# yxlao/deepSpeech

Measured on AMD Instinct MI355X. Metric: audio-sec/sec training throughput (whole node), DS2 BiGRU, higher is better.
Workload: dtype bf16; 1 GPU; model=DeepSpeech2 2xconv(32) + 5xBiGRU-800 bidirectional + CTC, global_batch=32, seq_len=1000, parallelism=dp1, engine=hip

## Files before the change

deepspeech_amd/csrc/api.h:

```cpp
#pragma once
#include <hip/hip_runtime_api.h>
#include <stddef.h>

extern "C" {

struct DS2Fill {
  int n;
  unsigned* ptr[8];
  unsigned long long words[8];
  unsigned pattern[8];
};

hipEvent_t ds2_take_stop_event();
void ds2_arm_stop_event(hipEvent_t e);

int ds2_multi_fill(int n, void* const* ptrs, const unsigned long long* bytes, const unsigned* patterns,
                   hipStream_t st);
int ds2_multi_copy(int n, void* const* dst, const void* const* src, const unsigned long long* rows,
                   const unsigned* src_row, const unsigned* dst_row, const unsigned* src_pitch,
                   const unsigned* dst_pitch, float* sdst, const float* svals, int ns, hipStream_t st);
int ds2_wait_resident(const unsigned* word, long long timeout, hipStream_t st);
int ds2_prep_inputs(const float* x, void* y, long long n, const int* lens_in, int* lens_out, int nl,
                    hipStream_t st);
int ds2_transpose_bf16(const void* in, void* out, int R, int C, int ldi, int ldo, hipStream_t st);
// ... 166 lines not shown

int ds2_bn_stats(const void* y, int y_bf16, int N, int C, int T, int F, float* part, int nb, float eps, float* mean,
                 float* invstd, float* run_mean, float* run_var, float momentum, hipStream_t st);
int ds2_bn_chunks(int N, int T, int F);
int ds2_bn_apply(const void* y, int y_bf16, const float* mean, const float* invstd, const float* gamma,
                 const float* beta, void* out, int out_bf16, int N, int C, int T, int F, int layout, hipStream_t st);
int ds2_bn_bwd(const void* dout, int dout_bf16, const void* y, int y_bf16, const float* mean, const float* invstd,
               const float* gamma, const float* beta, float* part, int nb, float* dgamma, float* dbeta, void* dy,
               int dy_bf16, int N, int C, int T, int F, int layout, hipStream_t st);

int ds2_adam_ema(float* p, const float* g, float* m, float* v, float* ema, void* p16, long long n, float lr_t,
                 float b1, float b2, float eps, float gscale, float ema_keep, const int* skip, int max_grid,
                 const float* hyper, int lds_reserve, hipStream_t st);
int ds2_adam_ema_ranges(float* p, const float* g, float* m, float* v, float* ema, void* p16, const long long* lohi,
                        int nr, float lr_t, float b1, float b2, float eps, float gscale, float ema_keep,
                        const float* hyper, hipStream_t st);
int ds2_grad_norm_blocks(long long n);
int ds2_grad_norm(const float* g, long long n, float gscale, float* part, int nblocks, int* bad, hipStream_t st);
int ds2_cast_bf16(const float* x, void* y, long long n, hipStream_t st);
int ds2_col_sum(int n, const float* const* in, float* const* out, const int* R, const int* B, const int* C,
                const int* acc, hipStream_t st);
int ds2_fc_bias_grad(const void* G, int M, int ldg, int K, const float* scale, float alpha, float* out, int acc,
                     hipStream_t st);
int ds2_hist_nbucket();
int ds2_hist_npos();
int ds2_hist_blocks(long long n);
int ds2_hist_stats(const void* x, int bf16, long long n, unsigned* counts, float* part, int blocks, hipStream_t st);
int ds2_spin(long long ticks, int blocks, int threads, int lds_bytes, int* done, hipStream_t st);

struct DS2Conv1WgradBn {
  const void *dz, *y1;
  const float *mean, *invstd, *gamma, *beta, *dbeta, *dgamma;
};

struct DS2Conv2DgradBn {
  const void* y1;
  const float *mean, *invstd, *gamma, *beta;
  float* part;
};

size_t ds2_conv2_fwd_smem(int F1);
size_t ds2_conv2_dgrad_smem(int F2);
size_t ds2_conv2_wgrad_smem(int F1);
long long ds2_conv2_wgrad_part_floats(int grid);
long long ds2_conv1_wgrad_part_floats(int grid);
int ds2_conv1_fwd_grid(int N, int T1);
int ds2_conv1_fwd(const void* x, const void* w, const float* bias, void* y, float* part, int N, int T, int F0,
                  int T1, int F1, hipStream_t st);
int ds2_conv2_fwd(const void* x, const void* w, const float* bias, void* y, float* part, int grid, int N, int T1,
                  int F1, int T2, int F2, long long* trace, hipStream_t st);
int ds2_conv2_dgrad(const void* dy, const void* w, void* dx, int grid, int N, int T1, int F1, int T2, int F2,
                    const DS2Conv2DgradBn* bn, long long* trace, hipStream_t st);
int ds2_conv2_wgrad(const void* dy, const void* x, float* part, int grid, float* dw, int N, int T1, int F1, int T2,
                    int F2, hipStream_t st);
int ds2_conv1_wgrad(const void* dy, const void* x, float* part, int grid, float* dw, int N, int T, int F0, int T1,
                    int F1, const DS2Conv1WgradBn* bn, hipStream_t st);
int ds2_bn_cl_finalize(const float* part, int nb, double M, float eps, float* mean, float* invstd, float* run_mean,
                       float* run_var, float momentum, hipStream_t st);
int ds2_bn_cl_apply(const void* y, const float* mean, const float* invstd, const float* gamma, const float* beta,
                    void* out, int N, int T, int F, int tmaj, hipStream_t st);
int ds2_bn_cl_bwd(const void* dz, const void* y, const float* mean, const float* invstd, const float* gamma,
                  const float* beta, float* part, int nb, float* dgamma, float* dbeta, void* dy, int N, int T, int F,
                  int tmaj, int part_ready, hipStream_t st);

struct DS2Feat {
  const void* pcm;
  long long row_stride;
  int S, lead, mode, B, T_max;
  const int* lens;
  const float* offset;
  const float* gain;
  const float* basis;
  const int* mel_idx;
  const float* mel_w;
  const float* dct;
  const float* lifter;
  void* out;
  int* frames;
};

int ds2_audio_stats(const void* pcm, int in_i16, long long row_stride, int S, int B, const int* lens, float* offset,
                    float* gain, hipStream_t st);
int ds2_featurize(const DS2Feat* a, int kind, int in_i16, int out_bf16, hipStream_t st);

}
```

deepspeech_amd/csrc/bindings.cpp:

```cpp
#include <torch/extension.h>
#include <c10/hip/HIPStream.h>
#include <hip/hip_runtime.h>

#include <cstdint>
#include <string>
#include <vector>

#include "api.h"

namespace {

using OptT = c10::optional<at::Tensor>;

hipStream_t cur_stream() { return c10::hip::getCurrentHIPStream().stream(); }

void check(int rc, const char* what) {
  TORCH_CHECK(rc == 0, "deepspeech_amd kernel launch failed in ", what, " (code ", rc, ")");
}

constexpr unsigned kLightEvent = hipEventDisableTiming;

int64_t event_new(unsigned flags) {
  hipEvent_t e = nullptr;
  TORCH_CHECK(hipEventCreateWithFlags(&e, flags ? flags : kLightEvent) == hipSuccess, "hipEventCreateWithFlags");
// ... 454 lines not shown

void conv1_fwd(at::Tensor x, at::Tensor w, OptT bias, at::Tensor y, at::Tensor part) {
  need_bf16(x, "x"); need_bf16(w, "w"); need_bf16(y, "y");
  TORCH_CHECK(x.dim() == 3 && y.dim() == 4 && y.size(3) == 32 && w.numel() == 32 * 100, "conv1_fwd shapes");
  const int N = (int)x.size(0), T = (int)x.size(1), F0 = (int)x.size(2), T1 = (int)y.size(1), F1 = (int)y.size(2);
  TORCH_CHECK(y.size(0) == N, "conv1_fwd batch");
  need_f32(part, "part", (int64_t)ds2_conv1_fwd_grid(N, T1) * 64);
  check(ds2_conv1_fwd(x.data_ptr(), w.data_ptr(), ptr_or_null<float>(bias, "bias"), y.data_ptr(),
                      part.data_ptr<float>(), N, T, F0, T1, F1, cur_stream()), "conv1_fwd");
}
int64_t conv1_fwd_grid(int64_t N, int64_t T1) { return ds2_conv1_fwd_grid((int)N, (int)T1); }

long long* trace_ptr(const OptT& trace) {
  if (!trace) return nullptr;
  TORCH_CHECK(trace->is_cuda() && trace->scalar_type() == at::kLong && trace->numel() >= 8 * 16 * 6 &&
                  trace->is_contiguous(), "trace must be a contiguous cuda int64 tensor of >= 768 elements");
  return reinterpret_cast<long long*>(trace->data_ptr<int64_t>());
}

void conv2_fwd(at::Tensor x, at::Tensor w, OptT bias, at::Tensor y, at::Tensor part, int64_t grid, OptT trace) {
  need_bf16(x, "x"); need_bf16(w, "w"); need_bf16(y, "y");
  TORCH_CHECK(x.dim() == 4 && y.dim() == 4 && x.size(3) == 32 && y.size(3) == 32 && w.numel() == 32 * 32 * 50,
              "conv2_fwd shapes");
  TORCH_CHECK(grid > 0, "grid");
  need_f32(part, "part", grid * 64);
  check(ds2_conv2_fwd(x.data_ptr(), w.data_ptr(), ptr_or_null<float>(bias, "bias"), y.data_ptr(),
                      part.data_ptr<float>(), (int)grid, (int)x.size(0), (int)x.size(1), (int)x.size(2),
                      (int)y.size(1), (int)y.size(2), trace_ptr(trace), cur_stream()), "conv2_fwd");
}

void conv2_dgrad(at::Tensor dy, at::Tensor w, at::Tensor dx, int64_t grid, OptT y1, OptT mean, OptT invstd,
                 OptT gamma, OptT beta, OptT part, OptT trace) {
  need_bf16(dy, "dy"); need_bf16(w, "w"); need_bf16(dx, "dx");
  TORCH_CHECK(dy.dim() == 4 && dx.dim() == 4 && dy.size(3) == 32 && dx.size(3) == 32 && w.numel() == 32 * 32 * 50,
              "conv2_dgrad shapes");
  TORCH_CHECK(grid > 0, "grid");
  DS2Conv2DgradBn bn{};
  const bool with_bn = y1.has_value();
  if (with_bn) {
    TORCH_CHECK(mean && invstd && gamma && beta && part, "conv2_dgrad: the BN arguments come all or none");
    need_bf16(*y1, "y1");
    TORCH_CHECK(y1->sizes() == dx.sizes(), "y1 must have dx's shape");
    need_f32(*mean, "mean", 32); need_f32(*invstd, "invstd", 32); need_f32(*gamma, "gamma", 32);
    need_f32(*beta, "beta", 32); need_f32(*part, "part", grid * 64);
    bn = DS2Conv2DgradBn{y1->data_ptr(), mean->data_ptr<float>(), invstd->data_ptr<float>(),
                         gamma->data_ptr<float>(), beta->data_ptr<float>(), part->data_ptr<float>()};
  }
  check(ds2_conv2_dgrad(dy.data_ptr(), w.data_ptr(), dx.data_ptr(), (int)grid, (int)dx.size(0), (int)dx.size(1),
                        (int)dx.size(2), (int)dy.size(1), (int)dy.size(2), with_bn ? &bn : nullptr,
                        trace_ptr(trace), cur_stream()),
        "conv2_dgrad");
}

void conv2_wgrad(at::Tensor dy, at::Tensor x, at::Tensor part, at::Tensor dw, int64_t grid) {
  need_bf16(dy, "dy"); need_bf16(x, "x");
  TORCH_CHECK(grid > 0, "grid");
  need_f32(part, "part", ds2_conv2_wgrad_part_floats((int)grid));
  need_f32(dw, "dw", 32 * 32 * 50);
  check(ds2_conv2_wgrad(dy.data_ptr(), x.data_ptr(), part.data_ptr<float>(), (int)grid, dw.data_ptr<float>(),
                        (int)x.size(0), (int)x.size(1), (int)x.size(2), (int)dy.size(1), (int)dy.size(2),
                        cur_stream()), "conv2_wgrad");
}

void conv1_wgrad(at::Tensor dy, at::Tensor x, at::Tensor part, at::Tensor dw, int64_t grid, OptT y1, OptT mean,
                 OptT invstd, OptT gamma, OptT beta, OptT dbeta, OptT dgamma) {
  need_bf16(dy, "dy"); need_bf16(x, "x");
  TORCH_CHECK(grid > 0, "grid");
  need_f32(part, "part", ds2_conv1_wgrad_part_floats((int)grid));
  need_f32(dw, "dw", 32 * 100);
  DS2Conv1WgradBn bn{};
  const bool with_bn = y1.has_value();
  if (with_bn) {
    TORCH_CHECK(mean && invstd && gamma && beta && dbeta && dgamma, "conv1_wgrad: the BN arguments come all or none");
    need_bf16(*y1, "y1");
    TORCH_CHECK(y1->sizes() == dy.sizes(), "y1 must have dz's shape");
    for (const OptT* t : {&mean, &invstd, &gamma, &beta, &dbeta, &dgamma}) need_f32(**t, "bn vector", 32);
    bn = DS2Conv1WgradBn{dy.data_ptr(), y1->data_ptr(), mean->data_ptr<float>(), invstd->data_ptr<float>(),
                         gamma->data_ptr<float>(), beta->data_ptr<float>(), dbeta->data_ptr<float>(),
                         dgamma->data_ptr<float>()};
  }
  check(ds2_conv1_wgrad(with_bn ? nullptr : dy.data_ptr(), x.data_ptr(), part.data_ptr<float>(), (int)grid,
                        dw.data_ptr<float>(), (int)x.size(0), (int)x.size(1), (int)x.size(2), (int)dy.size(1),
                        (int)dy.size(2), with_bn ? &bn : nullptr, cur_stream()), "conv1_wgrad");
}
int64_t conv2_wgrad_part_floats(int64_t grid) { return ds2_conv2_wgrad_part_floats((int)grid); }
int64_t conv1_wgrad_part_floats(int64_t grid) { return ds2_conv1_wgrad_part_floats((int)grid); }

void bn_cl_finalize(at::Tensor part, int64_t nb, double M, double eps, at::Tensor mean, at::Tensor invstd,
                    OptT run_mean, OptT run_var, double momentum) {
  need_f32(part, "part", nb * 64);
  need_f32(mean, "mean", 32); need_f32(invstd, "invstd", 32);
  check(ds2_bn_cl_finalize(part.data_ptr<float>(), (int)nb, M, (float)eps, mean.data_ptr<float>(),
                           invstd.data_ptr<float>(), ptr_or_null<float>(run_mean, "run_mean"),
                           ptr_or_null<float>(run_var, "run_var"), (float)momentum, cur_stream()), "bn_cl_finalize");
}

void bn_cl_apply(at::Tensor y, at::Tensor mean, at::Tensor invstd, at::Tensor gamma, at::Tensor beta, at::Tensor out,
                 bool tmaj) {
  need_bf16(y, "y"); need_bf16(out, "out");
  TORCH_CHECK(y.dim() == 4 && y.size(3) == 32 && out.numel() == y.numel(), "bn_cl_apply shapes");
  need_f32(mean, "mean", 32); need_f32(invstd, "invstd", 32); need_f32(gamma, "gamma", 32); need_f32(beta, "beta", 32);
  check(ds2_bn_cl_apply(y.data_ptr(), mean.data_ptr<float>(), invstd.data_ptr<float>(), gamma.data_ptr<float>(),
                        beta.data_ptr<float>(), out.data_ptr(), (int)y.size(0), (int)y.size(1), (int)y.size(2),
                        tmaj ? 1 : 0, cur_stream()), "bn_cl_apply");
}

void bn_cl_bwd(at::Tensor dz, at::Tensor y, at::Tensor mean, at::Tensor invstd, at::Tensor gamma, at::Tensor beta,
               at::Tensor part, int64_t nb, at::Tensor dgamma, at::Tensor dbeta, at::Tensor dy, bool tmaj,
               int64_t part_ready) {
  need_bf16(dz, "dz"); need_bf16(y, "y"); need_bf16(dy, "dy");
  TORCH_CHECK(y.dim() == 4 && y.size(3) == 32 && dz.numel() == y.numel() && dy.numel() == y.numel(),
              "bn_cl_bwd shapes");
  need_f32(part, "part", nb * 64);
  need_f32(mean, "mean", 32); need_f32(invstd, "invstd", 32); need_f32(gamma, "gamma", 32); need_f32(beta, "beta", 32);
// ... 697 lines not shown
  m.def("bn_bwd", &bn_bwd);
  m.def("adam_ema", &adam_ema, py::arg("p"), py::arg("g"), py::arg("m"), py::arg("v"), py::arg("ema"),
        py::arg("p16"), py::arg("lr_t"), py::arg("b1"), py::arg("b2"), py::arg("eps"), py::arg("gscale"),
        py::arg("ema_keep"), py::arg("skip"), py::arg("max_grid"), py::arg("hyper") = py::none(),
        py::arg("lds_reserve") = 0);
  m.def("adam_ema_ranges", &adam_ema_ranges, py::arg("p"), py::arg("g"), py::arg("m"), py::arg("v"),
        py::arg("ema"), py::arg("p16"), py::arg("lohi"), py::arg("lr_t"), py::arg("b1"), py::arg("b2"),
        py::arg("eps"), py::arg("gscale"), py::arg("ema_keep"), py::arg("hyper") = py::none());
  m.def("grad_norm_blocks", &grad_norm_blocks);
  m.def("grad_norm", &grad_norm);
  m.def("cast_bf16", &cast_bf16);
  m.def("device_info", &device_info);
  m.def("fp8_quant_blocks", &fp8_quant_blocks);
  m.def("prep_inputs", &prep_inputs);
  m.def("multi_copy", &multi_copy, py::arg("dsts"), py::arg("srcs"), py::arg("sdst") = py::none(),
        py::arg("svals") = std::vector<double>{});
  m.def("fp8_quant2", &fp8_quant2, py::arg("a"), py::arg("b"), py::arg("alpha"), py::arg("a8"), py::arg("b8"),
        py::arg("part"), py::arg("scales"), py::arg("a2") = py::none(), py::arg("asum") = py::none());
  m.def("transpose_bf16", &transpose_bf16);
  m.def("gemm8", &gemm8, py::arg("A"), py::arg("B"), py::arg("C"), py::arg("bias"), py::arg("epi"),
        py::arg("alpha") = 1.0, py::arg("alpha_dev") = py::none(), py::arg("alpha_dev2") = py::none(),
        py::arg("a_col") = false, py::arg("b_col") = false, py::arg("splits") = 1, py::arg("ws") = py::none(),
        py::arg("cnt") = py::none(), py::arg("max_grid") = 0, py::arg("fill") = std::vector<at::Tensor>{},
        py::arg("fill_pat") = std::vector<int64_t>{}, py::arg("ext_red") = false);
  m.def("gemm8_group", &gemm8_group, py::arg("A"), py::arg("B"), py::arg("C"), py::arg("epi"), py::arg("splits"),
        py::arg("a_col"), py::arg("b_col"), py::arg("ws"), py::arg("cnt"), py::arg("max_grid"));
  m.def("gemm8_splits", [](int64_t K, bool fp8, int64_t S) { return ds2_gemm8_splits((int)K, fp8 ? 1 : 0, (int)S); });
  m.def("multi_fill", &multi_fill);
  m.def("col_sum", &col_sum);
  m.def("wait_resident", &wait_resident);
  m.def("fc_bias_grad", &fc_bias_grad);
  m.def("ctc_beam", &ctc_beam);
  m.def("ctc_beam_backtrack", &ctc_beam_backtrack);
  m.def("ctc_beam_lm", &ctc_beam_lm);
  m.def("ctc_beam_backtrack_lm", &ctc_beam_backtrack_lm);
  m.def("event_new", &event_new, py::arg("flags") = 0);
  m.def("arm_stop_event", &arm_stop_event);
  m.def("disarm_stop_event", &disarm_stop_event);
  m.def("event_free", &event_free);
  m.def("event_record", &event_record);
  m.def("event_wait", &event_wait);
  m.def("event_query", &event_query);
  m.def("stream_wait", &stream_wait);
  m.def("ctc_greedy", &ctc_greedy, py::arg("logits"), py::arg("lens"), py::arg("labels"), py::arg("counts"),
        py::arg("blank"), py::arg("score") = py::none());
  m.def("conv1_fwd", &conv1_fwd);
  m.def("conv1_fwd_grid", &conv1_fwd_grid);
  m.def("conv2_fwd", &conv2_fwd, py::arg("x"), py::arg("w"), py::arg("bias"), py::arg("y"), py::arg("part"),
        py::arg("grid"), py::arg("trace") = py::none());
  m.def("conv2_dgrad", &conv2_dgrad, py::arg("dy"), py::arg("w"), py::arg("dx"), py::arg("grid"),
        py::arg("y1") = py::none(), py::arg("mean") = py::none(), py::arg("invstd") = py::none(),
        py::arg("gamma") = py::none(), py::arg("beta") = py::none(), py::arg("part") = py::none(),
        py::arg("trace") = py::none());
  m.def("conv2_wgrad", &conv2_wgrad);
  m.def("conv1_wgrad", &conv1_wgrad, py::arg("dy"), py::arg("x"), py::arg("part"), py::arg("dw"), py::arg("grid"),
        py::arg("y1") = py::none(), py::arg("mean") = py::none(), py::arg("invstd") = py::none(),
        py::arg("gamma") = py::none(), py::arg("beta") = py::none(), py::arg("dbeta") = py::none(),
        py::arg("dgamma") = py::none());
  m.def("conv2_wgrad_part_floats", &conv2_wgrad_part_floats);
  m.def("conv1_wgrad_part_floats", &conv1_wgrad_part_floats);
  m.def("bn_cl_finalize", &bn_cl_finalize);
  m.def("bn_cl_apply", &bn_cl_apply);
  m.def("bn_cl_bwd", &bn_cl_bwd, py::arg("dz"), py::arg("y"), py::arg("mean"), py::arg("invstd"), py::arg("gamma"),
        py::arg("beta"), py::arg("part"), py::arg("nb"), py::arg("dgamma"), py::arg("dbeta"), py::arg("dy"),
        py::arg("tmaj"), py::arg("part_ready") = 0);
  m.def("gemm", &gemm, py::arg("A"), py::arg("B"), py::arg("C"), py::arg("bias"), py::arg("M"), py::arg("N"),
        py::arg("K"), py::arg("a_col"), py::arg("b_col"), py::arg("epi"), py::arg("alpha"), py::arg("cfg"),
        py::arg("alpha_dev") = py::none(), py::arg("Ml") = 0, py::arg("Nl") = 0, py::arg("Kl") = 0,
        py::arg("fill") = std::vector<at::Tensor>{}, py::arg("fill_pat") = std::vector<int64_t>{});
  m.def("gemm_tile", &gemm_tile);
  m.def("head_ctc", &head_ctc, py::arg("h"), py::arg("W"), py::arg("bias"), py::arg("lens"), py::arg("labels"),
        py::arg("label_lens"), py::arg("loss"), py::arg("G"), py::arg("ws"), py::arg("blank"), py::arg("zero_inf"),
        py::arg("mean") = py::none(), py::arg("counter") = py::none(), py::arg("first_bad") = py::none());
  m.def("fc_logits", &fc_logits);
  m.def("audio_stats", &audio_stats, py::arg("pcm"), py::arg("lens"), py::arg("offset"), py::arg("gain"));
  m.def("featurize", &featurize, py::arg("pcm"), py::arg("lens"), py::arg("offset"), py::arg("gain"),
        py::arg("basis"), py::arg("mel_idx"), py::arg("mel_w"), py::arg("dct"), py::arg("lifter"), py::arg("kind"),
        py::arg("lead"), py::arg("mode"), py::arg("out"), py::arg("frames"));
  m.def("hist_stats", &hist_stats);
  m.def("hist_nbucket", []() { return ds2_hist_nbucket(); });
  m.def("hist_blocks", [](int64_t n) { return ds2_hist_blocks(n); });
  m.def("nonfinite_watch", &nonfinite_watch);
  m.def("spin", [](int64_t ticks, int64_t blocks, int64_t threads, int64_t lds_bytes, at::Tensor done) {
    need_gpu(done, "done");
    TORCH_CHECK(done.scalar_type() == at::kInt, "done: int32");
    check(ds2_spin(ticks, (int)blocks, (int)threads, (int)lds_bytes, done.data_ptr<int>(), cur_stream()), "spin");
  });
}
```

deepspeech_amd/csrc/conv_frontend.hip:

```cpp
#include "common.h"

using namespace ds2;

namespace {

typedef __attribute__((ext_vector_type(16))) float f32x16;
typedef __attribute__((ext_vector_type(4))) short s16x4;
typedef __attribute__((address_space(3))) void lds_void_t;
typedef __attribute__((address_space(3))) s16x4 lds_s16x4_t;

constexpr int CC = 32;
constexpr float CLIP = 20.0f;
constexpr int MT = 3;

__device__ __forceinline__ f32x16 mfma32(bf16x8 a, bf16x8 b, f32x16 c) {
  return __builtin_amdgcn_mfma_f32_32x32x16_bf16(a, b, c, 0, 0, 0);
}

__device__ __forceinline__ void glds16(const void* g, void* lds_wave_base) {
  __builtin_amdgcn_global_load_lds(g, (lds_void_t*)lds_wave_base, 16, 0, 0);
}

__device__ __forceinline__ unsigned swz(unsigned R, unsigned c) { return R * 64u + ((c ^ ((R >> 2) & 3u)) << 4); }

// ... 352 lines not shown
#pragma unroll
          for (int j = 0; j < 2; ++j)
#pragma unroll
            for (int e = 0; e < 4; ++e) {
              const int fo = (32 * m + 8 * (2 * kh + j) + e) * CC;
              yv[m][j][e] = m < 2 ? yb[fo] : yb[min(fo, lastoff)];
            }
      }
#pragma unroll
      for (int m = 0; m < MT; ++m)
#pragma unroll
        for (int j = 0; j < 2; ++j)
#pragma unroll
          for (int e = 0; e < 4; ++e) {
            const int f1 = 32 * m + 8 * (2 * kh + j) + 4 * hi + e;
            if (m < 2 || f1 < a.F1) {
              const bf16_t d = f2bf(own[m][j][e]);
              stg[f1 * CC + col] = d;
              if (bn) {
                const float xh = (bf2f(yv[m][j][e]) - bmu) * bis;
                const float zz = xh * bg + bbt;
                const float dd = (zz > 0.f && zz < CLIP) ? bf2f(d) : 0.f;
                bs += dd;
                bq += dd * xh;
              }
            }
          }
    }
    lds_barrier();
    if (out) {
      i32x4* dst = (i32x4*)(a.dx + rowoff);
      for (int q = kh * 64 + lane; q < a.F1 * 4; q += 128) dst[q] = ((const i32x4*)stg)[q];
    }
    c2_stamp(a.trace, it, 4);
    if (tile + per < t_hi) issue(tile + per);
    c2_stamp(a.trace, it, 5);
  }
  if (bn) {
    bs += __shfl_xor(bs, 32, 64);
    bq += __shfl_xor(bq, 32, 64);
    float* sh = (float*)red;
    __syncthreads();
    if (lane < 32) { sh[(w * 32 + lane) * 2] = bs; sh[(w * 32 + lane) * 2 + 1] = bq; }
    __syncthreads();
    if (tid < 64) a.part[(size_t)blockIdx.x * 64 + tid] = sh[tid] + sh[64 + tid] + sh[128 + tid] + sh[192 + tid];
  }
}

struct Conv2Wgrad {
  const bf16_t* dy;
  const bf16_t* x;
  float* part;
  int N, T1, F1, T2, F2;
};
constexpr int C2W_PAIRS = C2_KT * C2_KF;
constexpr int C2W_WAVES = 8;
constexpr int C2W_PPW = 7;

__global__ __launch_bounds__(512) void conv2_wgrad_kernel(Conv2Wgrad a) {
  extern __shared__ __attribute__((aligned(16))) unsigned char smem[];
  const int tid = threadIdx.x, lane = tid & 63, w = uni(tid >> 6);
  const int dyBytes = 80 * 64;
  const int xBytes = (9 * a.F1 + 84) * 64;
  const int bufBytes = dyBytes + xBytes;
  unsigned char* const buf0 = smem;
  unsigned char* const buf1 = smem + bufBytes;
  for (int b = 0; b < 2; ++b) {
    unsigned char* bb = b ? buf1 : buf0;
    for (int o = a.F2 * 64 + tid * 4; o < dyBytes; o += 512 * 4) *(unsigned*)(bb + o) = 0u;
    for (int o = 10 * a.F1 * 64 + tid * 4; o < xBytes; o += 512 * 4) *(unsigned*)(bb + dyBytes + o) = 0u;
  }
  const int ntiles = a.N * a.T2;
  const int dyChunks = a.F2 * 4, xChunks = 10 * a.F1 * 4;
  auto issue = [&](int t, unsigned char* dst) {
    const int n = t / a.T2, t2 = t - n * a.T2;
    const unsigned char* sdy = (const unsigned char*)(a.dy + ((size_t)n * a.T2 + t2) * a.F2 * CC);
    const unsigned char* sx = (const unsigned char*)(a.x + ((size_t)n * a.T1 + 2 * t2) * a.F1 * CC);
    for (int p0 = w * 64; p0 < dyChunks; p0 += 512) {
      const int p = p0 + lane;
      if (p < dyChunks) glds16(sdy + (size_t)p * 16, dst + (size_t)p0 * 16);
    }
    for (int p0 = w * 64; p0 < xChunks; p0 += 512) {
      const int p = p0 + lane;
      if (p < xChunks) glds16(sx + (size_t)p * 16, dst + dyBytes + (size_t)p0 * 16);
    }
  };
  const int g = lane >> 4, h = g >> 1, cb = (g & 1) * 16, q = (lane & 15) >> 2, pp = lane & 3;
  const unsigned lofs = (unsigned)((8 * h + q) * 64 + (cb + 4 * pp) * 2);
  const int npairs = (w < C2W_PAIRS - 6 * C2W_WAVES) ? 7 : 6;

  f32x16 acc[C2W_PPW];
#pragma unroll
  for (int i = 0; i < C2W_PPW; ++i) acc[i] = (f32x16){};
  __syncthreads();
  int it = 0;
  if ((int)blockIdx.x < ntiles) issue(blockIdx.x, buf0);
  for (int tile = blockIdx.x; tile < ntiles; tile += gridDim.x, ++it) {
    const unsigned char* cur = (it & 1) ? buf1 : buf0;
    asm volatile("s_waitcnt vmcnt(0)" ::: "memory");
    __syncthreads();
    if (tile + (int)gridDim.x < ntiles) issue(tile + gridDim.x, (it & 1) ? buf0 : buf1);
    const unsigned char* xs = cur + dyBytes;
#pragma unroll
    for (int kk = 0; kk < 5; ++kk) {
      const unsigned k0 = (unsigned)(16 * kk) * 64u;
      const bf16x8 av = cat8(tr_read(cur + k0 + lofs), tr_read(cur + k0 + lofs + 4 * 64));
#pragma unroll
      for (int i = 0; i < C2W_PPW; ++i) {
        if (i < npairs) {
          const int P = w + C2W_WAVES * i;
          const int kt = P / 5, kf = P - 5 * (P / 5);
          const unsigned rb = (unsigned)(kt * a.F1 + kf) * 64u + k0 + lofs;
          const bf16x8 bv = cat8(tr_read(xs + rb), tr_read(xs + rb + 4 * 64));
          acc[i] = mfma32(av, bv, acc[i]);
        }
      }
    }
  }
  f32x4* out = (f32x4*)(a.part + (size_t)blockIdx.x * C2W_PAIRS * 1024);
#pragma unroll
  for (int i = 0; i < C2W_PPW; ++i) {
    if (i < npairs) {
      const int P = w + C2W_WAVES * i;
#pragma unroll
      for (int r4 = 0; r4 < 4; ++r4)
        out[(P * 4 + r4) * 64 + lane] = (f32x4){acc[i][4 * r4], acc[i][4 * r4 + 1], acc[i][4 * r4 + 2], acc[i][4 * r4 + 3]};
    }
  }
}

template <int KIND>
__global__ __launch_bounds__(256) void wgrad_reduce_kernel(const float* __restrict__ part, int nb, int E,
                                                           float* __restrict__ dw) {
  __shared__ f32x4 sh[4][64];
  const int tid = threadIdx.x, g = tid >> 6, l = tid & 63;
  const int e4 = blockIdx.x * 64 + l, E4 = E >> 2;
  const f32x4* p4 = (const f32x4*)part;
  f32x4 s0 = {}, s1 = {};
  int b = g;
  for (; b + 4 < nb; b += 8) {
    s0 += p4[(size_t)b * E4 + e4];
    s1 += p4[(size_t)(b + 4) * E4 + e4];
  }
  if (b < nb) s0 += p4[(size_t)b * E4 + e4];
  sh[g][l] = s0 + s1;
  __syncthreads();
  if (g != 0) return;
  const f32x4 v = sh[0][l] + sh[1][l] + sh[2][l] + sh[3][l];
#pragma unroll
  for (int j = 0; j < 4; ++j) {
    const int e = e4 * 4 + j;
    const int P = e >> 10, rem = e & 1023, r4 = rem >> 8, ln = (rem >> 2) & 63;
    const int row = (rem & 3) + 8 * r4 + 4 * (ln >> 5), c = ln & 31;
    if (KIND == 0) {
      const int kt = P / 5, kf = P % 5;
      dw[((row * CC + c) * C2_KT + kt) * C2_KF + kf] = v[j];
    } else {
      const int kt = 4 * P + (c >> 3), kf = c & 7;
      if (kf < 5) dw[(row * 20 + kt) * 5 + kf] = v[j];
    }
  }
}

struct Conv1Fwd {
  const bf16_t* x;
  const bf16_t* w;
  const float* bias;
  bf16_t* y;
  float* part;
  int N, T, F0, T1, F1;
// ... 42 lines not shown
  __syncthreads();
  float ssum = 0.f, ssq = 0.f;
  const int t1 = t1_0 + w;
  if (t1 < a.T1) {
    f32x16 acc[MT];
#pragma unroll
    for (int m = 0; m < MT; ++m) acc[m] = (f32x16){};
#pragma unroll
    for (int s = 0; s < 10; ++s) {
      const int r = 2 * w + 2 * s + hi;
#pragma unroll
      for (int m = 0; m < MT; ++m) {
        const unsigned* p = (const unsigned*)(xs + r * C1_XS + 2 * (32 * m + col));
        const unsigned u0 = p[0], u1 = p[1], u2 = p[2], u3 = p[3];
        const bf16x8 av = __builtin_bit_cast(bf16x8, (i32x4){(int)u0, (int)u1, (int)u2, (int)u3});
        acc[m] = mfma32(av, bfr[s], acc[m]);
      }
    }
    bf16_t* yl = ys[w];
#pragma unroll
    for (int m = 0; m < MT; ++m)
#pragma unroll
      for (int r = 0; r < 16; ++r) {
        const int f1 = 32 * m + (r & 3) + 8 * (r >> 2) + 4 * hi;
        if (f1 < a.F1) {
          const bf16_t b = f2bf(acc[m][r] + bco);
          yl[f1 * CC + col] = b;
          const float vb = bf2f(b);
          ssum += vb;
          ssq += vb * vb;
        }
      }
    i32x4* dst = (i32x4*)(a.y + ((size_t)n * a.T1 + t1) * a.F1 * CC);
    for (int q = lane; q < a.F1 * 4; q += 64) dst[q] = ((const i32x4*)yl)[q];
  }
  write_stats(ssum, ssq, statsh, 4, a.part);
}

struct Conv1Wgrad {
  const bf16_t* dy;
  const bf16_t* x;
  float* part;
  int N, T, F0, T1, F1;
  const bf16_t *dz, *y1;
  const float *mean, *invstd, *gamma, *beta, *dbeta, *dgamma;
  float M;
};
constexpr int C1W_XP = 88;
constexpr int C1W_DY = C1_ROWS * 80 * 64;
constexpr int C1W_XD = C1_IN * 8 * C1W_XP * 2;
constexpr int C1W_RED = 4 * 5 * 4 * 64 * 16;
constexpr int C1W_RAW = C1_IN * C1_XS * 2;
constexpr int C1W_SMEM = (C1W_DY + C1W_XD + C1W_RAW) > C1W_RED ? (C1W_DY + C1W_XD + C1W_RAW) : C1W_RED;

__global__ __launch_bounds__(256) void conv1_wgrad_kernel(Conv1Wgrad a) {
  extern __shared__ __attribute__((aligned(16))) unsigned char smem[];
  const int tid = threadIdx.x, lane = tid & 63, w = uni(tid >> 6);
  const int hi = lane >> 5, col = lane & 31;
  unsigned char* dys = smem;
  bf16_t* xd = (bf16_t*)(smem + C1W_DY);
  bf16_t* raw = (bf16_t*)(smem + C1W_DY + C1W_XD);
  const int tb = (a.T1 + C1_ROWS - 1) / C1_ROWS;
  const int ntiles = a.N * tb;
  const int g = lane >> 4, h = g >> 1, cb = (g & 1) * 16, q = (lane & 15) >> 2, pp = lane & 3;
  const unsigned lofs = (unsigned)((8 * h + q) * 64 + (cb + 4 * pp) * 2);
  const int bkt = col >> 3, bkf = col & 7;

  const bool bn = a.dz != nullptr;
  float bmu[8], bis[8], bg[8], bbt[8], bmdb[8], bmdg[8];
  if (bn) {
#pragma unroll
    for (int j = 0; j < 8; ++j) {
      const int c = (tid & 3) * 8 + j;
      bmu[j] = a.mean[c]; bis[j] = a.invstd[c]; bg[j] = a.gamma[c]; bbt[j] = a.beta[c];
      bmdb[j] = a.dbeta[c] / a.M; bmdg[j] = a.dgamma[c] / a.M;
    }
  }
  f32x16 acc[5];
#pragma unroll
  for (int i = 0; i < 5; ++i) acc[i] = (f32x16){};
  for (int tile = blockIdx.x; tile < ntiles; tile += gridDim.x) {
    const int n = tile / tb, t1_0 = (tile - n * tb) * C1_ROWS;
    __syncthreads();
    for (int ch = tid; ch < C1_ROWS * 80 * 4; ch += 256) {
      const int r = ch / 320, rem = ch - r * 320, pos = rem >> 2, c4 = rem & 3;
      const int t1 = t1_0 + r;
      i32x4 v = (i32x4){0, 0, 0, 0};
      if (pos < a.F1 && t1 < a.T1) {
        const size_t off = (((size_t)n * a.T1 + t1) * a.F1 + pos) * CC + c4 * 8;
        if (bn) {
          const bf16x8 y = *(const bf16x8*)(a.y1 + off), d = *(const bf16x8*)(a.dz + off);
          bf16x8 o;
#pragma unroll
          for (int j = 0; j < 8; ++j) {
            const float xh = (bf2f((bf16_t)y[j]) - bmu[j]) * bis[j];
            const float zz = xh * bg[j] + bbt[j];
            const float dd = (zz > 0.f && zz < CLIP) ? bf2f((bf16_t)d[j]) : 0.f;
            o[j] = (short)f2bf(bg[j] * bis[j] * (dd - bmdb[j] - xh * bmdg[j]));
          }
          v = __builtin_bit_cast(i32x4, o);
        } else {
          v = *(const i32x4*)(a.dy + off);
        }
      }
      *(i32x4*)(dys + ch * 16) = v;
    }
    stage_rows(raw, a.x + (size_t)n * a.T * a.F0, 2 * t1_0, a.T, a.F0);
    __syncthreads();
    for (int ch = tid; ch < C1_IN * 8 * 10; ch += 256) {
      const int kf = ch & 7, q = ch >> 3, r = q / 10, p0 = (q - r * 10) * 8;
      bf16x8 v;
#pragma unroll
      for (int j = 0; j < 8; ++j) v[j] = (short)raw[r * C1_XS + min(2 * (p0 + j) + kf, C1_XS - 1)];
      *(bf16x8*)(xd + (r * 8 + kf) * C1W_XP + p0) = v;
    }
    __syncthreads();
    const int t1 = t1_0 + w;
    if (t1 < a.T1) {
#pragma unroll
      for (int kk = 0; kk < 5; ++kk) {
        const unsigned k0 = (unsigned)(16 * kk);
        const unsigned char* ab = dys + (w * 80 + k0) * 64 + lofs;
        const bf16x8 av = cat8(tr_read(ab), tr_read(ab + 4 * 64));
#pragma unroll
        for (int nt = 0; nt < 5; ++nt) {
          const int r = 2 * w + 4 * nt + bkt;
          const bf16x8 bv = *(const bf16x8*)(xd + (r * 8 + bkf) * C1W_XP + k0 + 8 * hi);
          acc[nt] = mfma32(av, bv, acc[nt]);
        }
      }
    }
  }
  __syncthreads();
  f32x4* red = (f32x4*)smem;
#pragma unroll
  for (int nt = 0; nt < 5; ++nt)
#pragma unroll
    for (int r4 = 0; r4 < 4; ++r4)
      red[((w * 5 + nt) * 4 + r4) * 64 + lane] =
          (f32x4){acc[nt][4 * r4], acc[nt][4 * r4 + 1], acc[nt][4 * r4 + 2], acc[nt][4 * r4 + 3]};
  __syncthreads();
  f32x4* out = (f32x4*)(a.part + (size_t)blockIdx.x * 5 * 1024);
  for (int e = tid; e < 5 * 4 * 64; e += 256) {
    f32x4 v = red[e];
    for (int wv = 1; wv < 4; ++wv) v += red[wv * 5 * 4 * 64 + e];
    out[e] = v;
  }
}

__global__ __launch_bounds__(256) void bn_cl_finalize_kernel(const float* __restrict__ part, int nb, double M,
                                                             float eps, float* mean, float* invstd, float* run_mean,
                                                             float* run_var, float momentum) {
  __shared__ double sh[2][4];
  const int c = blockIdx.x, tid = threadIdx.x;
  double s = 0.0, q = 0.0;
  for (int b = tid; b < nb; b += 256) {
    s += part[((size_t)b * 32 + c) * 2 + 0];
    q += part[((size_t)b * 32 + c) * 2 + 1];
  }
#pragma unroll
  for (int o = 32; o > 0; o >>= 1) {
    s += __shfl_xor(s, o, 64);
    q += __shfl_xor(q, o, 64);
  }
  if ((tid & 63) == 0) { sh[0][tid >> 6] = s; sh[1][tid >> 6] = q; }
  __syncthreads();
  if (tid == 0) {
// ... 213 lines not shown
#pragma unroll
    for (int k = 0; k < 4; ++k) o8[e + k * step] = one(v[k], d[k]);
  }
  for (; e < total; e += step) o8[e] = one(y8[e], d8[e]);
}

template <typename K>
int set_smem(K kernel, size_t bytes) {
  return (int)hipFuncSetAttribute(reinterpret_cast<const void*>(kernel), hipFuncAttributeMaxDynamicSharedMemorySize,
                                  (int)bytes);
}

int shape_ok(int T1, int F1, int T2, int F2) {
  if (F1 < 5 || F1 > 80 || F2 != F1 - 4) return -40;
  if (T1 < 10 || T2 != (T1 - 10) / 2 + 1) return -41;
  return 0;
}

}

extern "C" {

size_t ds2_conv2_fwd_smem(int) { return (size_t)C2F_SMEM; }
size_t ds2_conv2_dgrad_smem(int) { return (size_t)C2D_SMEM; }
size_t ds2_conv2_wgrad_smem(int F1) { return (size_t)2 * (80 * 64 + (9 * F1 + 84) * 64); }
long long ds2_conv2_wgrad_part_floats(int grid) { return (long long)grid * C2W_PAIRS * 1024; }
long long ds2_conv1_wgrad_part_floats(int grid) { return (long long)grid * 5 * 1024; }
int ds2_conv1_fwd_grid(int N, int T1) { return N * ((T1 + C1_ROWS - 1) / C1_ROWS); }

int ds2_conv2_fwd(const void* x, const void* w, const float* bias, void* y, float* part, int grid, int N, int T1,
                  int F1, int T2, int F2, long long* trace, hipStream_t st) {
  if (int e = shape_ok(T1, F1, T2, F2)) return e;
  const size_t smem = ds2_conv2_fwd_smem(F1);
  DS2_HIP_CHECK((hipError_t)set_smem(conv2_fwd_kernel, smem));
  Conv2Fwd a{(const bf16_t*)x, (const bf16_t*)w, bias, (bf16_t*)y, part, N, T1, F1, T2, F2, trace};
  hipLaunchKernelGGL(conv2_fwd_kernel, dim3(grid), dim3(256), smem, st, a);
  return (int)hipGetLastError();
}

int ds2_conv2_dgrad(const void* dy, const void* w, void* dx, int grid, int N, int T1, int F1, int T2, int F2,
                    const DS2Conv2DgradBn* bn, long long* trace, hipStream_t st) {
  if (int e = shape_ok(T1, F1, T2, F2)) return e;
  if (F1 <= 64) return -42;
  const size_t smem = ds2_conv2_dgrad_smem(F2);
  DS2_HIP_CHECK((hipError_t)set_smem(conv2_dgrad_kernel, smem));
  Conv2Dgrad a{(const bf16_t*)dy, (const bf16_t*)w, (bf16_t*)dx, N, T1, F1, T2, F2,
               bn ? (const bf16_t*)bn->y1 : nullptr, bn ? bn->mean : nullptr, bn ? bn->invstd : nullptr,
               bn ? bn->gamma : nullptr, bn ? bn->beta : nullptr, bn ? bn->part : nullptr, trace};
  hipLaunchKernelGGL(conv2_dgrad_kernel, dim3(grid), dim3(256), smem, st, a);
  return (int)hipGetLastError();
}

int ds2_conv2_wgrad(const void* dy, const void* x, float* part, int grid, float* dw, int N, int T1, int F1, int T2,
                    int F2, hipStream_t st) {
  if (int e = shape_ok(T1, F1, T2, F2)) return e;
  const size_t smem = ds2_conv2_wgrad_smem(F1);
  DS2_HIP_CHECK((hipError_t)set_smem(conv2_wgrad_kernel, smem));
  Conv2Wgrad a{(const bf16_t*)dy, (const bf16_t*)x, part, N, T1, F1, T2, F2};
  hipLaunchKernelGGL(conv2_wgrad_kernel, dim3(grid), dim3(512), smem, st, a);
  hipLaunchKernelGGL(wgrad_reduce_kernel<0>, dim3(C2W_PAIRS * 1024 / 256), dim3(256), 0, st, part, grid,
                     C2W_PAIRS * 1024, dw);
  return (int)hipGetLastError();
}

int ds2_conv1_fwd(const void* x, const void* w, const float* bias, void* y, float* part, int N, int T, int F0,
                  int T1, int F1, hipStream_t st) {
  if (F1 > 96 || F1 != (F0 - 5) / 2 + 1 || T1 != (T - 20) / 2 + 1 || T1 < 1) return -42;
  Conv1Fwd a{(const bf16_t*)x, (const bf16_t*)w, bias, (bf16_t*)y, part, N, T, F0, T1, F1};
  hipLaunchKernelGGL(conv1_fwd_kernel, dim3(ds2_conv1_fwd_grid(N, T1)), dim3(256), 0, st, a);
  return (int)hipGetLastError();
}

int ds2_conv1_wgrad(const void* dy, const void* x, float* part, int grid, float* dw, int N, int T, int F0, int T1,
                    int F1, const DS2Conv1WgradBn* bn, hipStream_t st) {
  if (F1 > 80 || F1 != (F0 - 5) / 2 + 1 || T1 != (T - 20) / 2 + 1 || T1 < 1) return -43;
  if ((dy == nullptr) == (bn == nullptr)) return -44;
  DS2_HIP_CHECK((hipError_t)set_smem(conv1_wgrad_kernel, C1W_SMEM));
  Conv1Wgrad a{(const bf16_t*)dy, (const bf16_t*)x, part, N, T, F0, T1, F1,
               bn ? (const bf16_t*)bn->dz : nullptr, bn ? (const bf16_t*)bn->y1 : nullptr,
               bn ? bn->mean : nullptr, bn ? bn->invstd : nullptr, bn ? bn->gamma : nullptr,
               bn ? bn->beta : nullptr, bn ? bn->dbeta : nullptr, bn ? bn->dgamma : nullptr,
               (float)((double)N * T1 * F1)};
  hipLaunchKernelGGL(conv1_wgrad_kernel, dim3(grid), dim3(256), C1W_SMEM, st, a);
  hipLaunchKernelGGL(wgrad_reduce_kernel<1>, dim3(5 * 1024 / 256), dim3(256), 0, st, part, grid, 5 * 1024, dw);
  return (int)hipGetLastError();
}

int ds2_bn_cl_finalize(const float* part, int nb, double M, float eps, float* mean, float* invstd, float* run_mean,
                       float* run_var, float momentum, hipStream_t st) {
  hipLaunchKernelGGL(bn_cl_finalize_kernel, dim3(CC), dim3(256), 0, st, part, nb, M, eps, mean, invstd, run_mean,
                     run_var, momentum);
  return (int)hipGetLastError();
}

int ds2_bn_cl_apply(const void* y, const float* mean, const float* invstd, const float* gamma, const float* beta,
                    void* out, int N, int T, int F, int tmaj, hipStream_t st) {
  if (F > 96) return -44;
  if (tmaj) {
    const int rows = N * T;
    hipLaunchKernelGGL(bn_cl_apply_tmaj_kernel, dim3(rows < 4096 ? rows : 4096), dim3(256), 0, st, (const bf16_t*)y,
                       mean, invstd, gamma, beta, (bf16_t*)out, N, T, F);
  } else {
    const long long nch = (long long)N * T * F * 4;
    long long nb = (nch + 255) / 256;
    if (nb > 8192) nb = 8192;
    hipLaunchKernelGGL(bn_cl_apply_kernel, dim3((unsigned)nb), dim3(256), 0, st, (const bf16_t*)y, mean, invstd,
                       gamma, beta, (bf16_t*)out, nch);
  }
  return (int)hipGetLastError();
}

// ... 19 lines not shown
```

Measured before the change: 41950 audio-sec/sec.

## Prefetch next conv1 wgrad tile into registers and permute-based x deinterleave

The conv1 weight-gradient kernel now loads the next tile's dy/dz/y1 and raw input rows into registers while the current tile is processed, which hides global-load latency behind the MFMA work. The stride-2 deinterleave of input rows into the shared-memory layout now uses 32-bit reads and byte permutes in place of per-element gathers. Optional trace timestamps are also added to the conv2 wgrad kernel. The register double-buffer raises VGPR pressure and could lower occupancy, and the unaligned-read edge handling adds complexity.

```diff
diff --git a/deepspeech_amd/csrc/api.h b/deepspeech_amd/csrc/api.h
--- a/deepspeech_amd/csrc/api.h
+++ b/deepspeech_amd/csrc/api.h
@@ -242,7 +242,7 @@
 int ds2_conv2_dgrad(const void* dy, const void* w, void* dx, int grid, int N, int T1, int F1, int T2, int F2,
                     const DS2Conv2DgradBn* bn, long long* trace, hipStream_t st);
 int ds2_conv2_wgrad(const void* dy, const void* x, float* part, int grid, float* dw, int N, int T1, int F1, int T2,
-                    int F2, hipStream_t st);
+                    int F2, long long* trace, hipStream_t st);
 int ds2_conv1_wgrad(const void* dy, const void* x, float* part, int grid, float* dw, int N, int T, int F0, int T1,
                     int F1, const DS2Conv1WgradBn* bn, hipStream_t st);
 int ds2_bn_cl_finalize(const float* part, int nb, double M, float eps, float* mean, float* invstd, float* run_mean,
diff --git a/deepspeech_amd/csrc/bindings.cpp b/deepspeech_amd/csrc/bindings.cpp
--- a/deepspeech_amd/csrc/bindings.cpp
+++ b/deepspeech_amd/csrc/bindings.cpp
@@ -530,14 +530,14 @@
         "conv2_dgrad");
 }
 
-void conv2_wgrad(at::Tensor dy, at::Tensor x, at::Tensor part, at::Tensor dw, int64_t grid) {
+void conv2_wgrad(at::Tensor dy, at::Tensor x, at::Tensor part, at::Tensor dw, int64_t grid, OptT trace) {
   need_bf16(dy, "dy"); need_bf16(x, "x");
   TORCH_CHECK(grid > 0, "grid");
   need_f32(part, "part", ds2_conv2_wgrad_part_floats((int)grid));
   need_f32(dw, "dw", 32 * 32 * 50);
   check(ds2_conv2_wgrad(dy.data_ptr(), x.data_ptr(), part.data_ptr<float>(), (int)grid, dw.data_ptr<float>(),
                         (int)x.size(0), (int)x.size(1), (int)x.size(2), (int)dy.size(1), (int)dy.size(2),
-                        cur_stream()), "conv2_wgrad");
+                        trace_ptr(trace), cur_stream()), "conv2_wgrad");
 }
 
 void conv1_wgrad(at::Tensor dy, at::Tensor x, at::Tensor part, at::Tensor dw, int64_t grid, OptT y1, OptT mean,
@@ -1341,7 +1341,8 @@
         py::arg("y1") = py::none(), py::arg("mean") = py::none(), py::arg("invstd") = py::none(),
         py::arg("gamma") = py::none(), py::arg("beta") = py::none(), py::arg("part") = py::none(),
         py::arg("trace") = py::none());
-  m.def("conv2_wgrad", &conv2_wgrad);
+  m.def("conv2_wgrad", &conv2_wgrad, py::arg("dy"), py::arg("x"), py::arg("part"), py::arg("dw"), py::arg("grid"),
+        py::arg("trace") = py::none());
   m.def("conv1_wgrad", &conv1_wgrad, py::arg("dy"), py::arg("x"), py::arg("part"), py::arg("dw"), py::arg("grid"),
         py::arg("y1") = py::none(), py::arg("mean") = py::none(), py::arg("invstd") = py::none(),
         py::arg("gamma") = py::none(), py::arg("beta") = py::none(), py::arg("dbeta") = py::none(),
diff --git a/deepspeech_amd/csrc/conv_frontend.hip b/deepspeech_amd/csrc/conv_frontend.hip
--- a/deepspeech_amd/csrc/conv_frontend.hip
+++ b/deepspeech_amd/csrc/conv_frontend.hip
@@ -428,6 +428,7 @@
   const bf16_t* x;
   float* part;
   int N, T1, F1, T2, F2;
+  long long* trace;
 };
 constexpr int C2W_PAIRS = C2_KT * C2_KF;
 constexpr int C2W_WAVES = 8;
@@ -473,9 +474,12 @@
   if ((int)blockIdx.x < ntiles) issue(blockIdx.x, buf0);
   for (int tile = blockIdx.x; tile < ntiles; tile += gridDim.x, ++it) {
     const unsigned char* cur = (it & 1) ? buf1 : buf0;
+    c2_stamp(a.trace, it, 0);
     asm volatile("s_waitcnt vmcnt(0)" ::: "memory");
     __syncthreads();
+    c2_stamp(a.trace, it, 1);
     if (tile + (int)gridDim.x < ntiles) issue(tile + gridDim.x, (it & 1) ? buf0 : buf1);
+    c2_stamp(a.trace, it, 2);
     const unsigned char* xs = cur + dyBytes;
 #pragma unroll
     for (int kk = 0; kk < 5; ++kk) {
@@ -492,6 +496,7 @@
         }
       }
     }
+    c2_stamp(a.trace, it, 3);
   }
   f32x4* out = (f32x4*)(a.part + (size_t)blockIdx.x * C2W_PAIRS * 1024);
 #pragma unroll
@@ -640,6 +645,97 @@
 constexpr int C1W_RED = 4 * 5 * 4 * 64 * 16;
 constexpr int C1W_RAW = C1_IN * C1_XS * 2;
 constexpr int C1W_SMEM = (C1W_DY + C1W_XD + C1W_RAW) > C1W_RED ? (C1W_DY + C1W_XD + C1W_RAW) : C1W_RED;
+constexpr int C1W_CK = C1_ROWS * 80 * 4 / 256;
+static_assert(C1W_CK * 256 == C1_ROWS * 80 * 4, "a tile's dy chunks divide evenly over the workgroup");
+constexpr int C1W_XG = 21;
+constexpr int C1W_XN = C1_IN * C1W_XG;
+constexpr int C1W_XI = (C1W_XN + 255) / 256;
+static_assert(8 * C1W_XG > 2 * 79 + 7 && 8 * C1W_XG <= C1_XS, "staged columns cover what is read");
+
+struct C1wTile {
+  i32x4 d[C1W_CK];
+  i32x4 y[C1W_CK];
+  i32x4 x[C1W_XI];
+  unsigned x4[C1W_XI];
+};
+
+__device__ __forceinline__ bool c1w_xitem(const Conv1Wgrad& a, int n, int t0, int it, int& r, int& g,
+                                          const bf16_t*& row, uintptr_t& lo, bool& odd) {
+  r = it / C1W_XG;
+  g = it - r * C1W_XG;
+  row = a.x + ((size_t)n * a.T + min(t0 + r, a.T - 1)) * a.F0;
+  const uintptr_t ad = (uintptr_t)(row + 8 * g);
+  lo = ad & ~(uintptr_t)3;
+  odd = (ad & 2) != 0;
+  return lo >= (uintptr_t)a.x && lo + 20 <= (uintptr_t)(a.x + (size_t)a.N * a.T * a.F0);
+}
+
+__device__ __forceinline__ bool c1w_chunk(int ch, int t1_0, int T1, int F1, int& t1, int& pos, int& c4) {
+  const int r = ch / 320, rem = ch - r * 320;
+  pos = rem >> 2;
+  c4 = rem & 3;
+  t1 = t1_0 + r;
+  return pos < F1 && t1 < T1;
+}
+
+__device__ __forceinline__ void c1w_load(C1wTile& t, const Conv1Wgrad& a, int tile, int tb, bool bn) {
+  const int n = tile / tb, t1_0 = (tile - n * tb) * C1_ROWS;
+#pragma unroll
+  for (int k = 0; k < C1W_CK; ++k) {
+    int t1, pos, c4;
+    c1w_chunk((int)threadIdx.x + 256 * k, t1_0, a.T1, a.F1, t1, pos, c4);
+    const size_t off = (((size_t)n * a.T1 + min(t1, a.T1 - 1)) * a.F1 + min(pos, a.F1 - 1)) * CC + c4 * 8;
+    if (bn) {
+      t.y[k] = *(const i32x4*)(a.y1 + off);
+      t.d[k] = *(const i32x4*)(a.dz + off);
+    } else {
+      t.d[k] = *(const i32x4*)(a.dy + off);
+    }
+  }
+#pragma unroll
+  for (int k = 0; k < C1W_XI; ++k) {
+    const int it = (int)threadIdx.x + 256 * k;
+    if (it >= C1W_XN) continue;
+    int r, g;
+    const bf16_t* row;
+    uintptr_t lo;
+    bool odd;
+    if (c1w_xitem(a, n, 2 * t1_0, it, r, g, row, lo, odd)) {
+      t.x[k] = *(const i32x4*)lo;
+      t.x4[k] = *(const unsigned*)(lo + 16);
+    } else {
+      bf16x8 v;
+#pragma unroll
+      for (int j = 0; j < 8; ++j) v[j] = (short)row[min(8 * g + j, a.F0 - 1)];
+      t.x[k] = __builtin_bit_cast(i32x4, v);
+      t.x4[k] = 0;
+    }
+  }
+}
+
+__device__ __forceinline__ void c1w_stage_x(bf16_t* raw, const C1wTile& t, const Conv1Wgrad& a, int n, int t0) {
+#pragma unroll
+  for (int k = 0; k < C1W_XI; ++k) {
+    const int it = (int)threadIdx.x + 256 * k;
+    if (it >= C1W_XN) continue;
+    int r, g;
+    const bf16_t* row;
+    uintptr_t lo;
+    bool odd;
+    const bool shift = c1w_xitem(a, n, t0, it, r, g, row, lo, odd) && odd;
+    const unsigned q[5] = {(unsigned)t.x[k][0], (unsigned)t.x[k][1], (unsigned)t.x[k][2], (unsigned)t.x[k][3],
+                           t.x4[k]};
+    i32x4 v;
+#pragma unroll
+    for (int i = 0; i < 4; ++i) {
+      const int c = 8 * g + 2 * i;
+      const unsigned wd = shift ? __builtin_amdgcn_alignbyte(q[i + 1], q[i], 2) : q[i];
+      const unsigned keep = (c < a.F0 ? 0xffffu : 0u) | (c + 1 < a.F0 ? 0xffff0000u : 0u);
+      v[i] = (int)(t0 + r < a.T ? wd & keep : 0u);
+    }
+    *(i32x4*)(raw + r * C1_XS + 8 * g) = v;
+  }
+}
 
 __global__ __launch_bounds__(256) void conv1_wgrad_kernel(Conv1Wgrad a) {
   extern __shared__ __attribute__((aligned(16))) unsigned char smem[];
@@ -667,17 +763,23 @@
   f32x16 acc[5];
 #pragma unroll
   for (int i = 0; i < 5; ++i) acc[i] = (f32x16){};
+  C1wTile cur, nxt;
+  if ((int)blockIdx.x < ntiles) c1w_load(nxt, a, blockIdx.x, tb, bn);
   for (int tile = blockIdx.x; tile < ntiles; tile += gridDim.x) {
     const int n = tile / tb, t1_0 = (tile - n * tb) * C1_ROWS;
+#pragma unroll
+    for (int i = 0; i < 5; ++i) asm volatile("" : "+a"(acc[i]));
+    cur = nxt;
+    if (tile + gridDim.x < (unsigned)ntiles) c1w_load(nxt, a, tile + gridDim.x, tb, bn);
     __syncthreads();
-    for (int ch = tid; ch < C1_ROWS * 80 * 4; ch += 256) {
-      const int r = ch / 320, rem = ch - r * 320, pos = rem >> 2, c4 = rem & 3;
-      const int t1 = t1_0 + r;
+#pragma unroll
+    for (int k = 0; k < C1W_CK; ++k) {
+      const int ch = tid + 256 * k;
+      int t1, pos, c4;
       i32x4 v = (i32x4){0, 0, 0, 0};
-      if (pos < a.F1 && t1 < a.T1) {
-        const size_t off = (((size_t)n * a.T1 + t1) * a.F1 + pos) * CC + c4 * 8;
+      if (c1w_chunk(ch, t1_0, a.T1, a.F1, t1, pos, c4)) {
         if (bn) {
-          const bf16x8 y = *(const bf16x8*)(a.y1 + off), d = *(const bf16x8*)(a.dz + off);
+          const bf16x8 y = __builtin_bit_cast(bf16x8, cur.y[k]), d = __builtin_bit_cast(bf16x8, cur.d[k]);
           bf16x8 o;
 #pragma unroll
           for (int j = 0; j < 8; ++j) {
@@ -688,19 +790,27 @@
           }
           v = __builtin_bit_cast(i32x4, o);
         } else {
-          v = *(const i32x4*)(a.dy + off);
+          v = cur.d[k];
         }
       }
       *(i32x4*)(dys + ch * 16) = v;
     }
-    stage_rows(raw, a.x + (size_t)n * a.T * a.F0, 2 * t1_0, a.T, a.F0);
+    c1w_stage_x(raw, cur, a, n, 2 * t1_0);
     __syncthreads();
-    for (int ch = tid; ch < C1_IN * 8 * 10; ch += 256) {
-      const int kf = ch & 7, q = ch >> 3, r = q / 10, p0 = (q - r * 10) * 8;
-      bf16x8 v;
-#pragma unroll
-      for (int j = 0; j < 8; ++j) v[j] = (short)raw[r * C1_XS + min(2 * (p0 + j) + kf, C1_XS - 1)];
-      *(bf16x8*)(xd + (r * 8 + kf) * C1W_XP + p0) = v;
+    constexpr int NI = C1_IN * 20 * 4;
+#pragma unroll
+    for (int k = 0; k < (NI + 255) / 256; ++k) {
+      const int it = tid + 256 * k;
+      if (it < NI) {
+        const int kf = 2 * (it & 3), q = it >> 2, r = q / 20, p0 = (q - r * 20) * 4;
+        const unsigned* src = (const unsigned*)(raw + r * C1_XS + 2 * p0 + kf);
+        const unsigned u0 = src[0], u1 = src[1], u2 = src[2], u3 = src[3];
+        unsigned* dst = (unsigned*)(xd + (r * 8 + kf) * C1W_XP + p0);
+        dst[0] = __builtin_amdgcn_perm(u1, u0, 0x05040100u);
+        dst[1] = __builtin_amdgcn_perm(u3, u2, 0x05040100u);
+        dst[C1W_XP / 2] = __builtin_amdgcn_perm(u1, u0, 0x07060302u);
+        dst[C1W_XP / 2 + 1] = __builtin_amdgcn_perm(u3, u2, 0x07060302u);
+      }
     }
     __syncthreads();
     const int t1 = t1_0 + w;
@@ -1020,11 +1130,11 @@
 }
 
 int ds2_conv2_wgrad(const void* dy, const void* x, float* part, int grid, float* dw, int N, int T1, int F1, int T2,
-                    int F2, hipStream_t st) {
+                    int F2, long long* trace, hipStream_t st) {
   if (int e = shape_ok(T1, F1, T2, F2)) return e;
   const size_t smem = ds2_conv2_wgrad_smem(F1);
   DS2_HIP_CHECK((hipError_t)set_smem(conv2_wgrad_kernel, smem));
-  Conv2Wgrad a{(const bf16_t*)dy, (const bf16_t*)x, part, N, T1, F1, T2, F2};
+  Conv2Wgrad a{(const bf16_t*)dy, (const bf16_t*)x, part, N, T1, F1, T2, F2, trace};
   hipLaunchKernelGGL(conv2_wgrad_kernel, dim3(grid), dim3(512), smem, st, a);
   hipLaunchKernelGGL(wgrad_reduce_kernel<0>, dim3(C2W_PAIRS * 1024 / 256), dim3(256), 0, st, part, grid,
                      C2W_PAIRS * 1024, dw);
```

New measurement: 42230 audio-sec/sec (median of 6 runs). No clear change (+0.7%).
